# wujian16/Cornell-MOE

Measured on AMD Instinct MI355X. Metric: q-KG gradient evals/s (n=1000,d=8,q=4,10k MC), higher is better.
Workload: dtype f64

## Files before the change

cornell_moe_amd/_lib.py:

```python
import ctypes as C
import os

_HERE = os.path.dirname(os.path.abspath(__file__))
LIB_PATH = os.environ.get("MOE_LIB_PATH") or os.path.join(_HERE, "lib", "libmoe_hip.so")

dp = C.POINTER(C.c_double)
ip = C.POINTER(C.c_int)

MOE_OK, MOE_ERR_RUNTIME, MOE_ERR_BOUNDS, MOE_ERR_INVALID_VALUE, MOE_ERR_SINGULAR = 0, 1, 2, 3, 4
COV_SQUARE_EXPONENTIAL, COV_MATERN_NU_2P5 = 0, 1


class MoeError(C.Structure):
    _fields_ = [("code", C.c_int), ("message", C.c_char * 480), ("payload", C.c_double * 3)]


class GdParams(C.Structure):
    _fields_ = [("num_multistarts", C.c_int), ("max_num_steps", C.c_int), ("max_num_restarts", C.c_int),
                ("num_steps_averaged", C.c_int), ("gamma", C.c_double), ("pre_mult", C.c_double),
                ("max_relative_change", C.c_double), ("tolerance", C.c_double), ("domain_type", C.c_int)]


class Prior(C.Structure):
    _fields_ = [("kind", C.c_int), ("a", C.c_double), ("b", C.c_double)]
# ... 134 lines not shown
    "moe_ll_destroy": (C.c_int, [C.c_void_p]),
    "moe_ll_evaluate": (C.c_int, [C.c_void_p, dp, C.c_int, dp, _EP]),
    "moe_ll_grad": (C.c_int, [C.c_void_p, dp, dp, _EP]),
    "moe_ll_set_objective": (C.c_int, [C.c_void_p, C.c_int, _EP]),
    "moe_ll_get_objective": (C.c_int, [C.c_void_p]),
    "moe_ll_loo_predict": (C.c_int, [C.c_void_p, dp, dp, dp, _EP]),
    "moe_ll_ascend": (C.c_int, [C.c_void_p, C.POINTER(GdParams), dp, dp, dp, _EP]),
    "moe_ll_multistart": (C.c_int, [C.c_void_p, C.POINTER(GdParams), dp, dp, C.c_int, dp, dp, ip, _EP]),
    "moe_ll_mcmc": (C.c_int, [C.c_void_p, C.POINTER(Prior), C.c_int, C.c_int, C.c_double, dp, dp, ip, dp, dp, dp, dp, dp, ip, _EP]),
    "moe_posterior_mean_optimize": (C.c_int, [_GP, C.c_int, C.POINTER(GdParams), dp, dp, dp, dp, _EP]),
    "moe_latin_hypercube": (C.c_int, [C.c_uint, dp, C.c_int, C.c_int, dp]),
    "moe_gp_mix_covariance": (C.c_int, [_GP, dp, C.c_int, ip, C.c_int, dp, _EP]),
    "moe_cov_build_probe": (C.c_int, [_GP, dp, C.c_int, C.c_int, dp, dp, _EP]),
    "moe_debug_cholesky": (C.c_int, [C.c_int, dp, C.c_int, dp, dp, ip, _EP]),
    "moe_debug_math": (C.c_int, [C.c_int, dp, C.c_int, dp, dp, _EP]),
    "moe_kxx_build_probe": (C.c_int, [_GP, C.c_int, dp, dp, _EP]),
    "moe_debug_fp64_rate": (C.c_int, [C.c_int, dp, _EP]),
    "moe_set_reference_quirks": (C.c_int, [C.c_int]),
    "moe_get_reference_quirks": (C.c_int, []),
    "moe_set_ensemble_launches": (C.c_int, [C.c_int]),
    "moe_ensemble_launch_stats": (C.c_int, [C.POINTER(C.c_longlong)]),
    "moe_last_kernel_ms": (C.c_int, [_GP, dp]),
    "moe_last_kernel_info": (C.c_int, [_GP, C.POINTER(C.c_int)]),
}

_lib = None


def load():
    global _lib
    if _lib is None:
        if not os.path.exists(LIB_PATH):
            raise ImportError("%s is missing: run `python -m cornell_moe_amd.build` (needs hipcc); there is no CPU fallback"
                              % LIB_PATH)
        lib = C.CDLL(LIB_PATH)
        for name, (res, args) in SIGNATURES.items():
            fn = getattr(lib, name)
            fn.restype = res
            fn.argtypes = args
        _lib = lib
    return _lib


def device_count():
    n = C.c_int(0)
    load().moe_device_count(C.byref(n))
# ... 7 lines not shown
```

cornell_moe_amd/api.py:

```python
import ctypes as C

import numpy as np

from . import _lib
from ._lib import dp, ip


class OptimalLearningException(Exception):
    pass


class BoundsException(OptimalLearningException):
    def __init__(self, message, value=0.0, min=0.0, max=0.0):
        super(BoundsException, self).__init__(message)
        self.value, self.min, self.max = value, min, max


class InvalidValueException(OptimalLearningException):
    def __init__(self, message, value=0.0, truth=0.0, tolerance=0.0):
        super(InvalidValueException, self).__init__(message)
        self.value, self.truth, self.tolerance = value, truth, tolerance


class SingularMatrixException(OptimalLearningException):
# ... 526 lines not shown
        x0, xp = _d(initial_guess)
        out = np.zeros(self.d - num_fidelity)
        val = C.c_double(0.0)
        err = _lib.MoeError()
        _check(_lib.load().moe_posterior_mean_optimize(self._h, int(num_fidelity), C.byref(g), bp, xp, out.ctypes.data_as(dp),
                                                       C.byref(val), C.byref(err)), err)
        return out, val.value

    def last_kernel_ms(self):
        out = np.zeros(5)
        _lib.load().moe_last_kernel_ms(self._h, out.ctypes.data_as(dp))
        return dict(mc=out[0], cov_build=out[1], tail=out[2], state=out[3], total=out[4])


    def last_kernel_info(self):
        out = (C.c_int * 8)()
        _lib.load().moe_last_kernel_info(self._h, out)
        keys = ("variant", "xlds", "waves", "tr", "weight_table", "fused_tail", "blocks", "prep")
        info = dict(zip(keys, [int(v) for v in out]))
        info["far_frame"], info["wide_frame"], info["lane"] = (info["xlds"] >> 1) & 1, (info["xlds"] >> 2) & 1, (info["xlds"] >> 3) & 1
        info["start_table"] = (info["xlds"] >> 4) & 1
        info["xlds"] &= 1
        return info


def kg_batch_multi(gps, shard, inner_params, bounds, discrete, Xq_all, Xp, num_mc, best_so_far, normals, want_grad=True,
                   num_fidelity=0):
    L = _lib.load()
    g0 = gps[0]
    gd = DeviceGP._gd(inner_params)
    bounds, bp = _d(bounds)
    discrete, dpp = _d(discrete)
    P = discrete.reshape(-1, g0.d - num_fidelity).shape[0]
    Xq_all = np.ascontiguousarray(Xq_all, dtype=np.float64)
    R, q, _ = Xq_all.shape
    if Xp is None or np.size(Xp) == 0:
        p, ppp = 0, None
    else:
        Xp, ppp = _d(Xp)
        p = Xp.reshape(-1, g0.d).shape[0]
    normals, npn = _d(normals)
    arr = (C.c_void_p * len(gps))(*[g._h.value for g in gps])
    kg = np.zeros(R)
    grad = np.zeros(R * q * g0.d)
    stats = _lib.KgStats()
    err = _lib.MoeError()
# ... 759 lines not shown
```

cornell_moe_amd/csrc/api.hip:

```cpp
#include <memory>
#include <algorithm>
#include <cmath>
#include <cstring>
#include <functional>
#include <mutex>
#include <random>
#include <string>
#include <condition_variable>
#include <thread>

#include "gp.hpp"
#include "kg.hpp"
#include "kg1_ascent.hpp"

struct moe_gp {
  moe::GpDev dev;
  std::mutex mu;
  moe_gp(const double* hyper, int cov_type, const double* X, const double* y, const double* noise, const int* derivs, int g,
         int d, int n, int device)
      : dev(hyper, cov_type, X, y, noise, derivs, g, d, n, device) {}
};

namespace {

// ... 497 lines not shown
    moe::DevBuf<double> dx, de, dr;
    dx.upload(x, n, nullptr);
    de.reserve(n);
    dr.reserve(n);
    moe::launch_debug_math(dx.p, n, de.p, dr.p, nullptr);
    de.download(exp_neg, n, nullptr);
    dr.download(sqrt_out, n, nullptr);
    MOE_HIP_CHECK(hipStreamSynchronize(nullptr));
  });
}

int moe_last_kernel_ms(const moe_gp_t* gp, double* out5) {
  if (gp == nullptr || out5 == nullptr) return MOE_ERR_RUNTIME;
  std::lock_guard<std::mutex> lk(const_cast<moe_gp_t*>(gp)->mu);
  for (int i = 0; i < 5; ++i) out5[i] = gp->dev.last_ms[i];
  return MOE_OK;
}

int moe_last_kernel_info(const moe_gp_t* gp, int* out8) {
  if (gp == nullptr || out8 == nullptr) return MOE_ERR_RUNTIME;
  std::lock_guard<std::mutex> lk(const_cast<moe_gp_t*>(gp)->mu);
  for (int i = 0; i < 8; ++i) out8[i] = gp->dev.last_info[i];
  return MOE_OK;
}

int moe_ei(const moe_gp_t* gp_c, const double* points_to_sample, const double* points_being_sampled, int num_to_sample,
           int num_being_sampled, int num_mc, double best_so_far, const double* normals, double* ei, double* grad_ei,
           moe_error_t* err) {
  return guarded(err, [&] {
    std::unique_lock<std::mutex> lk;
    moe::GpDev& gp = lock_gp(gp_c, lk);
    moe::ei_evaluate(gp, points_to_sample, points_being_sampled, num_to_sample, num_being_sampled, num_mc, best_so_far,
                     normals, ei, grad_ei);
  });
}

int moe_ei_batch(const moe_gp_t* gp_c, const double* points_to_sample_all, int num_evals, const double* points_being_sampled,
                 int num_to_sample, int num_being_sampled, int num_mc, double best_so_far, const double* normals,
                 double* ei, double* grad_ei, moe_error_t* err) {
  return guarded(err, [&] {
    std::unique_lock<std::mutex> lk;
    moe::GpDev& gp = lock_gp(gp_c, lk);
    moe::ei_evaluate_batch(gp, points_to_sample_all, num_evals, points_being_sampled, num_to_sample, num_being_sampled, num_mc,
                           best_so_far, normals, ei, grad_ei);
  });
}
// ... 1351 lines not shown
```

cornell_moe_amd/csrc/gp.hpp:

```cpp
#pragma once
#include <cstdlib>
#include <functional>
#include <memory>
#include <vector>

#include "common.hpp"
#include "host_math.hpp"
#include "kernels.hpp"

namespace moe {

void fill_cov_params(CovParams& cp, int cov_type, int d, const double* hyper);

struct GpDev {
  int device = 0;
  hipStream_t stream = nullptr;
  hipStream_t side_stream = nullptr;
  void release_side_streams();
  int d = 0, dp = 0, n = 0, g = 0, N = 0;
  long ldL = 0;
  const double* zeroed_L = nullptr;
  long zeroed_ld = 0;
  CovParams cp;
  DerivList derivs;
// ... 18 lines not shown
  DevBuf<double> kStateD;
  DevBuf<double> sMat, sOut;
  DevBuf<int> sInfo;
  DevBuf<double> lcbD;
  DevBuf<int> lcbI;
  DevBuf<double> looD;
  DevBuf<double> kg1D;
  DevBuf<int> kg1I;
  int kg1LastC = 0;
  DevBuf<double> kg1oD;
  DevBuf<int> kg1oI;
  DevBuf<double> ehviD;
  DevBuf<double> recD;
  DevBuf<int> recI;
  DevBuf<double> pmmD;
  DevBuf<int> pmmI;
  DevBuf<double> pathD;
  DevBuf<int> pathI;
  int num_cu = 256;
  double x_mean[kMaxDimPadded] = {0}, x_ext[kMaxDimPadded] = {0};
  void refresh_extent();
  double last_ms[5] = {0, 0, 0, 0, 0};
  int last_info[8] = {0, 0, 0, 0, 0, 0, 0, 0};

  GpDev(const double* hyper, int cov_type, const double* X_in, const double* y_in, const double* noise_in,
        const int* derivs_in, int g_in, int d_in, int n_in, int device_in);
  ~GpDev();
  GpDev(const GpDev&) = delete;
  GpDev& operator=(const GpDev&) = delete;

  void use_device() const;
  void set_covariance(const double* hyper);
  void rebuild();
  void add_points(const double* pts, const double* vals, int k);
  void add_points_unchecked(const double* pts, const double* vals, int k);
  void finish_factorisation();
  void set_hyperparameters(const double* hyper, const double* noise_in);
  double log_marginal_likelihood();
  void grad_log_marginal_likelihood(double* grad);
  std::vector<double> padded(const double* pts, int k) const;
  void mean_of_points(const double* pts, int k, double* mu, double* grad);
};

struct StateDev {
  StateLayout lay;
  bool have_W = false;
// ... 142 lines not shown
```

cornell_moe_amd/csrc/kg.hip:

```cpp
#include "kg.hpp"

#include <algorithm>
#include <array>
#include <memory>
#include <optional>
#include <chrono>
#include <cmath>
#include <cstdlib>

#include "kg_mc.hpp"
#include "kg_prep.hpp"
#include "kg_state.hpp"
#include "kg_tail.hpp"

namespace moe {

static thread_local int t_ens_members_hint = 1;
int ensemble_members_hint() { return t_ens_members_hint; }
void set_ensemble_members_hint(int members) { t_ens_members_hint = members > 1 ? members : 1; }


namespace {

struct EventTimer {
  hipEvent_t a = nullptr, b = nullptr;
  bool on = false;
  EventTimer() = default;
  EventTimer(const EventTimer&) = delete;
  EventTimer& operator=(const EventTimer&) = delete;
  ~EventTimer() {
    if (a != nullptr) (void)hipEventDestroy(a);
    if (b != nullptr) (void)hipEventDestroy(b);
  }
  void start(hipStream_t s) {
    on = Recorder::current() == nullptr;
    if (!on) return;
    if (a == nullptr) {
      MOE_HIP_CHECK(hipEventCreate(&a));
      MOE_HIP_CHECK(hipEventCreate(&b));
    }
    MOE_HIP_CHECK(hipEventRecord(a, s));
  }
  void stop(hipStream_t s) {
    if (on) MOE_HIP_CHECK(hipEventRecord(b, s));
  }
// ... 68 lines not shown
}

struct McPlan {
  int G = 0;
  int ntiles = 0;
  int variant = 0;
  bool xlds = true;
  bool far_frame = false;
  bool wide_frame = false;
  bool small_lane = false;
  bool lane_kernel = false;
  int waves = 0, blocks = 0;
  size_t shm = 0;
  int tr = -1, num_lds_tiles = 0;
  int wide_lds_tiles = 0;
  int pair_rows = 0;
  int rec_head = 0;
  int multi_trial = 0;
  bool prep = false;
  bool start_table = false;
  bool weight_table = false;
  long v_stride = 0;
  int v_slots1 = 0;
  bool fused_tail = false;
  int chunk_len = 0;
};

McPlan plan_mc(const GpDev& gp, const KgDims& k, const double* bounds, const double* Xq_all, const double* Xp, double weight_table_gb) {
  const double max_radius2 = (double)env_int("MOE_KG_DOT_MAX_RADIUS2", 10000);
  const bool lane_on = env_int("MOE_KG_LANE", 1) != 0;
  const long small_lane_max_samples = env_int("MOE_KG_SMALL_LANE_MAX_SAMPLES", 1024);
  const bool small_multi = env_int("MOE_KG_SMALL_MULTI", 1) != 0;
  const std::optional<int> forced_tr = env_opt("MOE_KG_TR");
  const std::optional<int> forced_variant = env_opt("MOE_KG_VARIANT");
  const int prep_mode = env_int("MOE_KG_PREP", -1);
  const bool stream_weights = env_int("MOE_KG_STREAM_WEIGHTS", 1) != 0;
  const double v_cap = std::getenv("MOE_KG_V_MAX_GB") ? (double)env_int("MOE_KG_V_MAX_GB", 4)
                                                      : (weight_table_gb >= 0.0 ? weight_table_gb : 4.0);
  McPlan pl;
  pl.fused_tail = fused_tail_taken(k.want_grad, k.g, k.m);

  const int d = k.d, dp = k.dp, n = k.n, g = k.g, m = k.m, u = k.u, A = k.A, E = k.E, num_local = k.num_local;
  const bool wide_dp = dp > 16;
  const int G = wide_dp ? (g == 0 ? 0 : (g <= 4 ? 4 : (g <= 8 ? 8 : 12))) : (g <= 4 ? g : (g <= 8 ? 8 : 12));
  const int ntiles = (n + u + 63) / 64;

  const size_t tab_bytes = sizeof(double) * (size_t)ntiles * (dp + 1) * 64;
  const size_t slab_bytes = sizeof(double) * ((size_t)ntiles * (1 + G) * 64 + 2 * kMaxM);
  const size_t slab_stream_bytes = slab_bytes + (mc::wide_eval(dp, false) ? sizeof(double) * mc::kWideScratch : 0);
  const size_t pad_bytes = sizeof(double) * (size_t)(1 + G) * 64;
  const size_t fixed_bytes = sizeof(double) * (kExpTabLen + (size_t)mc::kCstRows * dp);
  const size_t lds_max = 160 * 1024 - fixed_bytes - pad_bytes;
  bool xlds = true;
  bool wide_frame = false, far_frame = false;
  {
    double rad2 = 0.0;
    for (int kk = 0; kk < d; ++kk) {
      const double c = gp.x_mean[kk];
      double ext = gp.x_ext[kk];
// ... 92 lines not shown
  }
  if (ensemble_members_hint() > 1 && variant != 1 && blocks >= E && waves > 0) {
    const long tickets = 4;
    const long kb = std::max<long>(1, (num_local + tickets * waves - 1) / (tickets * waves));
    blocks = (int)std::min<long>(blocks, kb * E);
  }

  pl.G = G;
  pl.ntiles = ntiles;
  pl.variant = variant;
  pl.xlds = xlds;
  pl.far_frame = far_frame;
  pl.wide_frame = wide_frame;
  pl.small_lane = small_lane;
  pl.lane_kernel = lane_kernel;
  pl.waves = waves;
  pl.blocks = blocks;
  pl.shm = shm;
  pl.tr = tr;
  pl.num_lds_tiles = num_lds_tiles;
  pl.wide_lds_tiles = wide_lds_tiles;
  pl.pair_rows = (wide_dp || variant == 2 || (variant == 0 && mc::wide_eval(dp, xlds))) ? 1 : 0;
  pl.rec_head = rec_head;
  pl.multi_trial = (far_frame || small_lane) ? 0 : 1;
  if (small_lane && !far_frame && variant == 0 && lane_kernel && dp == 4 && small_multi) pl.multi_trial = 2;
  pl.prep = m > kMaxM || (prep_mode != 0 && (variant >= 1 || prep_mode == 1));
  pl.v_stride = (variant == 2) ? v_stride_tiles : k.N;
  pl.v_slots1 = (variant == 2) ? 1 + G : k.g1;
  pl.weight_table = variant >= 1 && pl.prep && 8.0 * (double)pl.v_stride * (double)num_local / 1e9 <= v_cap;
  if (variant == 2 && !(pl.weight_table && pl.prep))
    throw Error(MOE_ERR_RUNTIME, "streamed-weights MC kernel selected without its weight table");
  pl.chunk_len = tail_chunk_len(pl.fused_tail, m);
  pl.start_table = variant == 0 && xlds && g == 0 && G == 0;
  return pl;
}

TabParams table_rows(const GpDev& gp, const KgDims& k, int G, const double* Xq_all, const double* Xp, const double* disc_head) {
  const int d = k.d;
  TabParams tp;
  std::vector<int> order;
  std::vector<bool> used(kMaxDimPadded, false);
  for (int a = 0; a < k.g; ++a) {
    if (used[gp.derivs.idx[a]]) throw Error(MOE_ERR_INVALID_VALUE, "duplicate derivative index", gp.derivs.idx[a], 0, 0);
    order.push_back(gp.derivs.idx[a]);
    used[gp.derivs.idx[a]] = true;
  }
// ... 172 lines not shown
  mp.max_num_restarts = gd.max_num_restarts;
  mp.gamma = gd.gamma;
  mp.pre_mult = gd.pre_mult;
  mp.max_relative_change = gd.max_relative_change;
  if (k.simplex && mp.max_relative_change == 1.0) mp.max_relative_change -= 4.0 * 2.220446049250313e-16;
  mp.simplex = k.simplex ? 1 : 0;
  mp.inv_sqrt_size = 1.0 / std::sqrt((double)k.size);
  for (int r = 0; r < kMaxDimPadded; ++r) mp.inv_perm[r] = 0;
  for (int r = 0; r < kMaxDimPadded; ++r)
    if (tp.perm[r] >= 0 && tp.perm[r] < kMaxDimPadded) mp.inv_perm[tp.perm[r]] = r;
  mp.tolerance = gd.tolerance;
  mp.best_point = gp.kBestPoint.p;
  mp.best_value = gp.kBestValue.p;
  mp.beta = gp.kBeta.p;
  mp.counters = gp.kCounters.p;
  mp.next_sample = reinterpret_cast<unsigned int*>(gp.kCounters.p + (((size_t)2 * E + 15) / 16) * 16);
  mp.prof = gp.kCounters.p + n_ctr - 16;
  mp.best_j = nullptr;
  mp.V = nullptr;
  mp.v_stride = pl.v_stride;
  mp.v_slots1 = pl.v_slots1;
  mp.start_tab = nullptr;
  mp.start_stride = 0;
  if (pl.start_table) {
    mp.start_stride = (long)k.A * (1 + m) * (dp + 1);
    gp.kStartTab.reserve((size_t)mp.start_stride * E);
    double* start_tab_p = gp.kStartTab.p;
    launch_start_table(mp, dp, start_tab_p, s);
    mp.start_tab = start_tab_p;
  }
  t_state.stop(s);
  t_mc.start(s);
  const long total = (long)E * num_local;
  if (pl.prep) {
    gp.kBestJ.reserve((size_t)total);
    mp.best_j = gp.kBestJ.p;
    launch_sample_prep(mp, gp.kBestJ.p, gp.num_cu, s);
  }
  if (pl.weight_table) {
    gp.kV.reserve((size_t)mp.v_stride * (size_t)total + (size_t)64 * mp.v_slots1);
    memset_async(gp.kBeta.p + (size_t)total * m, 0, sizeof(double) * 64, s);
    mp.V = gp.kV.p;
    launch_sample_weights(mp, gp.kV.p, s, pl.variant == 2);
  }
  if (pl.variant == 0 && pl.lane_kernel)
    launch_mc_lane(mp, dp, pl.G, pl.rec_head, pl.blocks, pl.waves, pl.shm, s);
// ... 275 lines not shown
  gp.kBeta.reserve((size_t)E * num_local * m + 64);
  const size_t n_ctr = (size_t)2 * E + (size_t)E * (kTicketStride / 2) + 32;
  gp.kCounters.reserve(n_ctr);
  const int out_stride = 1 + m * m + 2 * k.ngrad;
  gp.kOut.reserve((size_t)out_stride * E);
  const bool sw_free = pl.fused_tail && fused_tail_sw_free();
  if (want_grad) {
    const int chunks = (num_local + pl.chunk_len - 1) / pl.chunk_len;
    if (!pl.fused_tail) gp.kT.reserve((size_t)N * E * num_local);
    if (!sw_free) gp.kC.reserve((size_t)E * num_local * m);
    gp.kTB.reserve((size_t)E * (chunks + 1) * m * N + (size_t)E * k.ngrad * kDirSlices + (sw_free ? (size_t)E * chunks * m * m : 0));
  }

  launch_xs_tab(gp.dX.p, k.n, gp.dUnion, u, dp, pl.ntiles, tp, gp.kTab.p, tab_stride, pl.pair_rows, gp.kCounters.p, (long)n_ctr, E, s);

  const KgMcParams mp = launch_mc_step(gp, k, pl, gd, tp, R, dBlobP, dNormalsP, se.bl, tab_stride, n_ctr, t_state, t_mc, s);
  {
    const int info[8] = {pl.variant,
                         ((pl.variant == 0 && pl.xlds) ? 1 : 0) | (pl.far_frame ? 2 : 0) | (pl.wide_frame ? 4 : 0) | (pl.lane_kernel ? 8 : 0) |
                             (pl.start_table ? 16 : 0),
                         pl.waves, pl.variant == 1 ? pl.tr : pl.wide_lds_tiles, pl.weight_table ? 1 : 0, pl.fused_tail ? 1 : 0, pl.blocks,
                         pl.prep ? 1 : 0};
    std::copy(info, info + 8, gp.last_info);
  }

  const KgTailParams tl = launch_tail_step(gp, k, pl, mp, R, dBlobP, dNormalsP, se.bl, dFin, out_stride, t_cov, t_tail, s);
  if (want_grad) {
    launch_grad_finish(gp, k, sp, tl, R, dBlobP, dFin, out_stride, sw_free, s);
    t_tail.stop(s);
  }
  return enqueue_results(gp, k, dFin, n_ctr, want_best_points, timers, wall0, s);
}

int kg_max_batch(const GpDev& gp, int P, int q, int p, int num_local, bool want_grad, double budget_gb) {
  const double N = gp.N, g1 = 1 + gp.g, u = q + p, m = u * g1, A = u + P;
  const double ngrad = want_grad ? q * g1 * gp.d : 0.0;
  const bool fused = fused_tail_taken(want_grad, gp.g, (int)m);
  const double chunks = std::ceil((double)num_local / tail_chunk_len(fused, (int)m));
  double doubles = N * (m + ngrad + A) + 3.0 * N * m + (double)num_local * (gp.dp + 1 + 2 * m) +
                   (want_grad ? (double)q * gp.d * m * (m + 1) / 2 : 0.0);
  if (want_grad) doubles += (fused ? 0.0 : N * (double)num_local) + (chunks + 1.0) * m * N;
  if (want_grad && !fused) doubles += 9.0 * m * (double)num_local;
  const double slots1 = gp.g <= 4 ? g1 : (gp.g <= 8 ? 9.0 : 13.0);
  doubles += (gp.n + u + 64.0) * slots1 * (double)num_local;
  doubles += 8.0 * N * m + (m * m + A * (1.0 + m + gp.d) + u * gp.dp + 8.0);
  const double per_eval_gb = 8.0 * doubles / 1e9;
// ... 33 lines not shown
```

cornell_moe_amd/csrc/kg_mc.hpp:

```cpp
#pragma once
#include <hip/hip_runtime.h>

#include "fastmath.hpp"
#include "kernels.hpp"

namespace moe {

#ifndef MOE_BLOCK_PROF
#define MOE_BLOCK_PROF 0
#endif
#if MOE_BLOCK_PROF
#define MOE_PROF_T(var) const unsigned long long var = __builtin_amdgcn_s_memtime()
#define MOE_PROF_ADD(dst, a, b) dst += (b) - (a)
#else
#define MOE_PROF_T(var)
#define MOE_PROF_ADD(dst, a, b)
#endif
constexpr int kTicketStride = 32;
constexpr int kMaxM = 64;
constexpr int kMaxMB = 128;
constexpr int kExpTabLen = 64;

struct KgRec {
  int L;
// ... 23 lines not shown
  const double* KinvY;
  const double* W;
  long w_stride;
  const double* blob;
  KgRec rec;
  const double* bounds;
  unsigned int free_mask;
  const double* normals;
  int first_sample, num_local;
  int max_num_steps, max_num_restarts;
  double gamma, pre_mult, max_relative_change, tolerance;
  double* best_point;
  double* best_value;
  double* beta;
  unsigned long long* counters;
  unsigned int* next_sample;
  unsigned long long* prof;
  const double* V;
  long v_stride;
  int v_slots1;
  const int* best_j;
  const double* start_tab;
  long start_stride;
};

#if defined(__HIPCC__)
namespace mc {

template <int DP> void launch_dp(const KgMcParams& P, int G, bool xlds, int blocks, int waves, size_t shm, hipStream_t s);
template <int DP> void launch_lane_dp(const KgMcParams& P, int G, int rec_head, int blocks, int waves, size_t shm, hipStream_t s);
template <int DP> void launch_stream_dp(const KgMcParams& P, int G, int blocks, int waves, size_t shm, hipStream_t s);
template <int DP> void launch_block_dp(const KgMcParams& P, int G, int tr, int num_lds_tiles, int blocks, int waves, hipStream_t s);

template <int CTRL, int ROW_MASK, bool FULL>
__device__ __forceinline__ double dpp_move(double v) {
  const int slo = __double2loint(v), shi = __double2hiint(v);
  int lo, hi;
  if (FULL) {
    lo = __builtin_amdgcn_mov_dpp(slo, CTRL, ROW_MASK, 0xf, false);
    hi = __builtin_amdgcn_mov_dpp(shi, CTRL, ROW_MASK, 0xf, false);
  } else {
    lo = __builtin_amdgcn_update_dpp(0, slo, CTRL, ROW_MASK, 0xf, false);
    hi = __builtin_amdgcn_update_dpp(0, shi, CTRL, ROW_MASK, 0xf, false);
  }
  return __hiloint2double(hi, lo);
}

// ... 729 lines not shown
      const double* Cj = C_disc + (long)j * m;
      for (int c0 = 0; c0 < m; c0 += 8) {
        double cv[8];
#pragma unroll
        for (int i = 0; i < 8; ++i) cv[i] = Cj[min(c0 + i, m - 1)];
#pragma unroll
        for (int i = 0; i < 8; ++i) v = fma(cv[i], (c0 + i < m) ? zb[min(c0 + i, kMaxM - 1)] : 0.0, v);
      }
      fj = -v;
    }
    double wmax = fj;
#pragma unroll
    for (int off = 32; off > 0; off >>= 1) wmax = fmax(wmax, __shfl_xor(wmax, off, 64));
    const unsigned long long ballot = __ballot(fj == wmax);
    const int first_lane = __ffsll((long long)ballot) - 1;
    if (wmax > best_f) {
      best_f = wmax;
      best_j = j0 + first_lane;
    }
  }
  return __builtin_amdgcn_readfirstlane(best_j);
}

}

inline size_t kg_mc_block_lds_bytes(int dp, int G, int num_lds_tiles) {
  return sizeof(double) * (mc::kBlockFixed + (size_t)num_lds_tiles * (dp + 1 + G) * 64);
}
inline size_t kg_mc_lane_fixed_bytes(int dp, int rec_head) {
  return sizeof(double) * ((size_t)kExpTabLen + (size_t)mc::kLaneCstRows * dp + (size_t)((rec_head + 1) & ~1));
}

#endif

}
```

cornell_moe_amd/csrc/kg_mc_block.hpp:

```cpp
#pragma once
#include "kg_mc.hpp"
#include "kg_mc_lds.hpp"

namespace moe {
namespace mc {


template <int DP, int G, bool WG, int COV>
__device__ __forceinline__ void point_terms(const double (&cx)[DP], const double (&cw)[1 + G], const double (&xq)[DP],
                                            const double* __restrict__ etab, double& accf, double (&accg)[DP],
                                            double (&accd)[G > 0 ? G : 1]) {
  double diff[DP];
  double r2 = 1.0e-300;
#pragma unroll
  for (int k = 0; k < DP; ++k) {
    diff[k] = cx[k] - xq[k];
    r2 = fma(diff[k], diff[k], r2);
  }
  double base, first, second;
  radial3<COV, (WG || G > 0), (WG && G > 0)>(r2, etab, base, first, second);
  double sd = 0.0;
  if (G > 0) {
#pragma unroll
    for (int a = 0; a < G; ++a) sd = fma(cw[1 + a], diff[a], sd);
// ... 489 lines not shown
    double* ldsw = ldsx + (long)num_lds_tiles * DP * 64;
    const int lane = threadIdx.x & 63;
    const int wave = threadIdx.x >> 6;
    const int nw = blockDim.x >> 6;
    const int m = P.m;
    const int size = P.dim - P.f;
    const int TL = num_lds_tiles;
    const int per = (TL + nw - 1) / nw;
    const int tl0 = min(wave * per, TL), tl1 = min(tl0 + per, TL);
    if (threadIdx.x < kExpTabLen) etab[threadIdx.x] = kExp2Tab64[threadIdx.x];
    BlockEval<DP, G, TR> ev;
    ev.xl = ldsx + (long)tl0 * DP * 64 + lane;
    ev.wl = ldsw + (long)tl0 * (1 + G) * 64 + lane;
    ev.ntl = tl1 - tl0;
    ev.etab = etab;
    ev.part = part;
    ev.inv_lp = P.inv_lp;
    ev.mean = P.mean;
    ev.nw = nw;
    ev.wave = wave;
    ev.lane = lane;
    ev.cov_type = P.cov_type;
    ev.par = 0;
    for (int e = blockIdx.x % P.E; e < P.E; e += (gridDim.x < (unsigned)P.E ? gridDim.x : P.E)) {
      const double* tab = P.XsTab + (long)e * P.tab_stride;
      const double* rec = P.blob + (long)e * P.rec.stride;
      const double* Lsm = rec + P.rec.L;
      const double* We = P.W + (long)e * P.w_stride;
      __syncthreads();
      if constexpr (DP > 16) {
        for (int t = threadIdx.x; t < TL * DP * 64; t += blockDim.x) {
          const int l = t & 63, r = (t >> 6) % DP, tile = (t >> 6) / DP;
          ldsx[t] = tab[(((long)tile * (DP / 2) + (r >> 1)) * 64 + l) * 2 + (r & 1)];
        }
      } else {
        for (int t = threadIdx.x; t < TL * DP * 64; t += blockDim.x) ldsx[t] = tab[t];
      }
  #pragma unroll
      for (int t = 0; t < TR; ++t) {
        const int tile = TL + wave * TR + t;
  #pragma unroll
        for (int k = 0; k < DP; ++k) ev.cx[t][k] = (tile < P.ntiles) ? tab[((long)tile * DP + k) * 64 + lane] : 0.0;
      }
  #if MOE_BLOCK_PROF
      unsigned long long p_tick = 0, p_setup = 0, p_w = 0, p_ls = 0, p_zb = 0, p_scan = 0;
  #endif
      while (true) {
// ... 83 lines not shown
          if (P.best_j == nullptr && lane < m) P.beta[so * m + lane] = bc;
        }
      }
  #if MOE_BLOCK_PROF
      if (threadIdx.x == 0) {
        atomicAdd(&P.prof[0], p_tick);
        atomicAdd(&P.prof[1], p_setup);
        atomicAdd(&P.prof[2], p_w);
        atomicAdd(&P.prof[3], p_ls);
        atomicAdd(&P.prof[4], ev.c_acc);
        atomicAdd(&P.prof[5], ev.c_red);
        atomicAdd(&P.prof[6], ev.c_bar);
        atomicAdd(&P.prof[7], ev.c_post);
        atomicAdd(&P.prof[8], ev.c_n);
        atomicAdd(&P.prof[9], ev.c_gtot);
        atomicAdd(&P.prof[10], ev.c_gn);
        atomicAdd(&P.prof[11], p_zb);
        atomicAdd(&P.prof[12], p_scan);
        atomicAdd(&P.prof[13], ev.seg[0]);
        atomicAdd(&P.prof[14], ev.seg[1]);
        atomicAdd(&P.prof[15], ev.seg[2] + ev.seg[3]);
      }
  #endif
      if (gridDim.x >= (unsigned)P.E) break;
    }
  }
};
template <int DP, int G, int TR>
__global__ __launch_bounds__(512) void kg_mc_block_kernel(KgMcParams P, int num_lds_tiles) {
  kg_mc_block_kernel_body<DP, G, TR>::run(MOE_VBLOCK, MOE_VGRID, nullptr, P, num_lds_tiles);
}

template <int DP, int G, int TR>
inline void launch_block_inst(const KgMcParams& P, int num_lds_tiles, int blocks, int waves, hipStream_t s) {
  const size_t shm = sizeof(double) * (kBlockFixed + (size_t)num_lds_tiles * (DP + 1 + G) * 64);
  auto kern = kg_mc_block_kernel<DP, G, TR>;
  launch_kernel_ens<kg_mc_block_kernel_body<DP, G, TR>, 512>(kern, dim3(blocks), dim3(waves * 64), shm, s, P, num_lds_tiles);
  MOE_HIP_CHECK(hipGetLastError());
}

template <int DP, int G>
inline void launch_block_g(const KgMcParams& P, int tr, int num_lds_tiles, int blocks, int waves, hipStream_t s) {
  switch (tr) {
    case 0: return launch_block_inst<DP, G, 0>(P, num_lds_tiles, blocks, waves, s);
    case 2: if constexpr (DP <= 16) return launch_block_inst<DP, G, 2>(P, num_lds_tiles, blocks, waves, s); break;
    case 4: if constexpr (DP <= 16) return launch_block_inst<DP, G, 4>(P, num_lds_tiles, blocks, waves, s); break;
  }
// ... 23 lines not shown
```

cornell_moe_amd/csrc/kg_mc_lane.hpp:

```cpp
#pragma once
#include "kg_mc.hpp"

namespace moe {
namespace mc {

constexpr int kLaneMaxThreads = 512;
constexpr int kLaneGradUnroll = 4;

template <int DP, int G, bool EXACT>
constexpr bool kLaneLookupFirst = DP <= 8 && G <= 1 && !EXACT;

constexpr int kMaxLaneDP = 16;

template <int DP>
__device__ __forceinline__ void fill_lane_constants(const KgMcParams& P, double* __restrict__ cst) {
  const int r = threadIdx.x;
  if (r < DP) {
    const double sc = P.inv_lp[r];
    cst[r] = sc;
    cst[DP + r] = (sc != 0.0) ? 1.0 / sc : 0.0;
    cst[2 * DP + r] = P.center[r];
    cst[3 * DP + r] = (P.perm[r] < P.dim) ? 1.0 : 0.0;
    cst[4 * DP + r] = P.bounds[2 * r];
    cst[5 * DP + r] = P.bounds[2 * r + 1];
// ... 443 lines not shown
  tot_val += n_val;
  tot_grad += n_grad;
  if (in_l) P.best_point[so * DP + perm_l] = xo_l;
  if (lane < m) P.beta[so * m + lane] = bc;
}

template <int DP, int G, bool EXACT = false, bool LF = false>
struct kg_mc_lane_kernel_body {
static __device__ __forceinline__ void run(const VIdx blockIdx, const VIdx gridDim, const void* argbase, const KgMcParams& P, int rec_head) {
  extern __shared__ __attribute__((aligned(16))) double smem[];
  const int lane = threadIdx.x & 63;
  const int wave = threadIdx.x >> 6;
  const int ntiles = P.ntiles;
  const int tab = ntiles * (DP + 1) * 64;
  const int wslab = ntiles * (1 + G) * 64 + 2 * kMaxM;
  double* cst = smem + kExpTabLen;
  double* rc = cst + kLaneCstRows * DP;
  double* coords = rc + rec_head;
  double* wshared = coords + tab;
  double* aw = wshared + wave * wslab;
  double* zb = aw + ntiles * (1 + G) * 64;
  if (threadIdx.x < kExpTabLen) smem[threadIdx.x] = kExp2Tab64[threadIdx.x];
  fill_lane_constants<DP>(P, cst);
  for (int e = blockIdx.x % P.E; e < P.E; e += (gridDim.x < (unsigned)P.E ? gridDim.x : P.E)) {
    const double* xg = P.XsTab + (long)e * P.tab_stride;
    __syncthreads();
    for (int pt = threadIdx.x; pt < ntiles * 64; pt += blockDim.x) {
      const int tl = pt >> 6, l = pt & 63;
      const double* src = xg + (long)tl * DP * 64 + l;
      double* dst = coords + tl * (DP + 1) * 64 + l;
      double xx = 0.0;
#pragma unroll
      for (int k = 0; k < DP; ++k) {
        const double v = src[k * 64];
        dst[k * 64] = v;
        xx = fma(v, v, xx);
      }
      dst[DP * 64] = xx;
    }
    {
      const double* rec = P.blob + (long)e * P.rec.stride;
      for (int i = threadIdx.x; i < rec_head; i += blockDim.x) rc[i] = rec[i];
    }
    __syncthreads();
    unsigned int ticket = 0;
    unsigned int* next = P.next_sample + (long)e * kTicketStride;
    if (lane == 0) ticket = atomicAdd(next, 1u);
    unsigned int tot_val = 0, tot_grad = 0;
    while (true) {
      const unsigned int sl = (unsigned int)__builtin_amdgcn_readfirstlane((int)ticket);
      if (sl >= (unsigned int)P.num_local) break;
      if (lane == 0) ticket = atomicAdd(next, 1u);
      const __attribute__((address_space(4))) KgMcParams* Pk = (const __attribute__((address_space(4))) KgMcParams*)argbase;
      asm volatile("" : "+s"(Pk));
      kg_sample_lane<DP, G, EXACT, LF>(*(const KgMcParams*)Pk, e, (int)sl, coords, aw, zb, smem, cst, rc, lane, tot_val, tot_grad);
    }
    if (lane == 0 && (tot_val | tot_grad) != 0) {
      atomicAdd(&P.counters[2 * e], (unsigned long long)tot_val);
      atomicAdd(&P.counters[2 * e + 1], (unsigned long long)tot_grad);
    }
    if (gridDim.x >= (unsigned)P.E) break;
  }
}
};
template <int DP, int G, bool EXACT = false>
__global__ __launch_bounds__(kLaneMaxThreads) void kg_mc_lane_kernel(KgMcParams P, int rec_head) {
  kg_mc_lane_kernel_body<DP, G, EXACT, kLaneLookupFirst<DP, G, EXACT>>::run(MOE_VBLOCK, MOE_VGRID, (const void*)__builtin_amdgcn_kernarg_segment_ptr(), P, rec_head);
}

template <int DP, int G, bool EXACT = false>
inline void launch_lane_inst(const KgMcParams& P, int rec_head, int blocks, int waves, size_t shm, hipStream_t s) {
  auto kern = kg_mc_lane_kernel<DP, G, EXACT>;
  launch_kernel_ens<kg_mc_lane_kernel_body<DP, G, EXACT>, kLaneMaxThreads>(kern, dim3(blocks), dim3(waves * 64), shm, s, P, rec_head);
  MOE_HIP_CHECK(hipGetLastError());
}

template <int DP, int G>
inline void launch_lane_g(const KgMcParams& P, int rec_head, int blocks, int waves, size_t shm, hipStream_t s) {
  if constexpr (DP == 4) {
    if (P.multi_trial == 2) return launch_lane_inst<DP, G, true>(P, rec_head, blocks, waves, shm, s);
  }
  launch_lane_inst<DP, G>(P, rec_head, blocks, waves, shm, s);
}

// ... 17 lines not shown
```

cornell_moe_amd/csrc/kg_mc_stream.hpp:

```cpp
#pragma once
#include "kg_mc.hpp"
#include "kg_mc_lds.hpp"

namespace moe {
namespace mc {

template <int DP, int G>
struct kg_mc_stream_kernel_body {
  static __device__ __forceinline__ void run(const VIdx blockIdx, const VIdx gridDim, const void*, const KgMcParams& P) {
    extern __shared__ __attribute__((aligned(16))) double smem[];
    const int lane = threadIdx.x & 63;
    const int wave = threadIdx.x >> 6;
    const int wtab = P.wide_lds_tiles * DP * 64;
    double* coords = smem + kExpTabLen;
    double* st = coords + wtab + wave * kWideScratch;
    if (threadIdx.x < kExpTabLen) smem[threadIdx.x] = kExp2Tab64[threadIdx.x];
    const int size = P.dim - P.f;
    for (int e = blockIdx.x % P.E; e < P.E; e += (gridDim.x < (unsigned)P.E ? gridDim.x : P.E)) {
      const double* xs = P.XsTab + (long)e * P.tab_stride;
      const double* rec = P.blob + (long)e * P.rec.stride;
      __syncthreads();
      {
        const d2t* src = reinterpret_cast<const d2t*>(xs);
        d2t* dst = reinterpret_cast<d2t*>(coords);
        for (int i = threadIdx.x; i < wtab / 2; i += blockDim.x) dst[i] = src[i];
      }
      __syncthreads();
      unsigned int ticket = 0;
      unsigned int* next = P.next_sample + (long)e * kTicketStride;
      if (lane == 0) ticket = atomicAdd(next, 1u);
      unsigned long long tot_val = 0, tot_grad = 0;
      while (true) {
        const unsigned int sl = (unsigned int)__builtin_amdgcn_readfirstlane((int)ticket);
        if (sl >= (unsigned int)P.num_local) break;
        if (lane == 0) ticket = atomicAdd(next, 1u);
        const long so = (long)e * P.num_local + sl;
        const int best_j = P.best_j[so];
        const double* disc = rec + P.rec.disc;
        double x[DP];
  #pragma unroll
        for (int k = 0; k < DP; ++k) x[k] = (k < size) ? disc[(long)best_j * size + k] : ((k < P.dim) ? 1.0 : 0.0);
        const d2t* xg = reinterpret_cast<const d2t*>(xs) + lane;
        lds_pair_ptr xl = (lds_pair_ptr)coords + lane;
        WideEval<DP, G, true> ev{xg, xl, {P.V + so * P.v_stride + (long)lane * (1 + G)}, smem, st + kLsRows * kMaxDimPadded,
                                 P.ntiles, P.wide_lds_tiles, P.cov_type, lane, P.mean};
        unsigned long long n_val = 0, n_grad = 0;
        const double fcur = line_search_lds<DP, G>(P, ev, st, x, n_val, n_grad);
        if (lane == 0) P.best_value[so] = fcur;
        tot_val += n_val;
        tot_grad += n_grad;
        if (lane < DP) {
          double v = 0.0;
  #pragma unroll
          for (int k = 0; k < DP; ++k)
            if (lane == k) v = x[k];
          P.best_point[so * DP + lane] = v;
        }
      }
      if (lane == 0 && (tot_val | tot_grad) != 0) {
        atomicAdd(&P.counters[2 * e], tot_val);
        atomicAdd(&P.counters[2 * e + 1], tot_grad);
      }
      if (gridDim.x >= (unsigned)P.E) break;
    }
  }
};
template <int DP, int G>
__global__ __launch_bounds__(512) void kg_mc_stream_kernel(KgMcParams P) {
  kg_mc_stream_kernel_body<DP, G>::run(MOE_VBLOCK, MOE_VGRID, nullptr, P);
}

template <int DP, int G>
inline void launch_stream_inst(const KgMcParams& P, int blocks, int waves, size_t shm, hipStream_t s) {
  auto kern = kg_mc_stream_kernel<DP, G>;
  launch_kernel_ens<kg_mc_stream_kernel_body<DP, G>, 512>(kern, dim3(blocks), dim3(waves * 64), shm, s, P);
  MOE_HIP_CHECK(hipGetLastError());
}

template <int DP>
void launch_stream_dp(const KgMcParams& P, int G, int blocks, int waves, size_t shm, hipStream_t s) {
  switch (G) {
    case 0: return launch_stream_inst<DP, 0>(P, blocks, waves, shm, s);
    case 1: if constexpr (DP <= 16) return launch_stream_inst<DP, 1>(P, blocks, waves, shm, s); break;
    case 2: if constexpr (DP <= 16) return launch_stream_inst<DP, 2>(P, blocks, waves, shm, s); break;
    case 3: if constexpr (DP <= 16) return launch_stream_inst<DP, 3>(P, blocks, waves, shm, s); break;
    case 4: return launch_stream_inst<DP, 4>(P, blocks, waves, shm, s);
// ... 9 lines not shown
```

cornell_moe_amd/csrc/kg_mc_wave.hpp:

```cpp
#pragma once
#include "kg_mc.hpp"
#include "kg_mc_lds.hpp"

namespace moe {
namespace mc {

template <int DP, int G, bool SMALL, bool XL>
struct WaveEval {
  const double* __restrict__ xs;
  const double* __restrict__ aw;
  const double* __restrict__ etab;
  int ntiles, cov_type;
  double mean;
  int lane;
  double* __restrict__ scr;
#if MOE_BLOCK_PROF
  unsigned long long c_v = 0, c_g = 0, n_v = 0, n_g = 0;
#endif
  __device__ __forceinline__ double eval_grad_frame(const double (&xf)[DP], double (&gradf)[DP]) {
#if MOE_BLOCK_PROF
    const unsigned long long t0 = __builtin_amdgcn_s_memtime();
#endif
    const double f = eval_pass<DP, G, true, SMALL, XL>(xs, aw, etab, ntiles, cov_type, mean, xf, gradf, lane, scr);
#if MOE_BLOCK_PROF
// ... 388 lines not shown
      if (lane == k) v = x[k];
    P.best_point[so * DP + lane] = v;
  }
  if (!prepped && lane < m) P.beta[so * m + lane] = bc;
}

template <int DP, int G, bool XLDS, bool SMALL>
struct kg_mc_kernel_body {
  static __device__ __forceinline__ void run(const VIdx blockIdx, const VIdx gridDim, const void*, const KgMcParams& P) {
    extern __shared__ __attribute__((aligned(16))) double smem[];
    const int lane = threadIdx.x & 63;
    const int wave = threadIdx.x >> 6;
    const int ntiles = P.ntiles;
    const int tab = ntiles * (DP + 1) * 64;
    const int wslab = ntiles * (1 + G) * 64 + 2 * kMaxM + (wide_eval(DP, XLDS) ? kWideScratch : 0);
    double* cst = smem + kExpTabLen;
    double* coords = cst + kCstRows * DP;
    const int wtab = wide_eval(DP, XLDS) ? P.wide_lds_tiles * DP * 64 : 0;
    double* aw = coords + (XLDS ? tab : wtab) + wave * wslab;
    double* zb = aw + ntiles * (1 + G) * 64;
    if (threadIdx.x < kExpTabLen) smem[threadIdx.x] = kExp2Tab64[threadIdx.x];
    fill_frame_constants<DP>(P, cst);
    if (!XLDS) __syncthreads();
    for (int e = blockIdx.x % P.E; e < P.E; e += (gridDim.x < (unsigned)P.E ? gridDim.x : P.E)) {
      const double* xs = P.XsTab + (long)e * P.tab_stride;
      if (XLDS) {
        __syncthreads();
        for (int pt = threadIdx.x; pt < ntiles * 64; pt += blockDim.x) {
          const int tl = pt >> 6, l = pt & 63;
          const double* src = xs + (long)tl * DP * 64 + l;
          double* dst = coords + tl * (DP + 1) * 64 + l;
          double xx = 0.0;
  #pragma unroll
          for (int k = 0; k < DP; ++k) {
            const double v = src[k * 64];
            dst[k * 64] = v;
            xx = fma(v, v, xx);
          }
          dst[DP * 64] = xx;
        }
        xs = coords;
        __syncthreads();
      }
      if constexpr (wide_eval(DP, XLDS)) {
        __syncthreads();
        const d2t* src = reinterpret_cast<const d2t*>(xs);
        d2t* dst = reinterpret_cast<d2t*>(coords);
        for (int i = threadIdx.x; i < wtab / 2; i += blockDim.x) dst[i] = src[i];
        __syncthreads();
      }
      unsigned int ticket = 0;
      unsigned int* next = P.next_sample + (long)e * kTicketStride;
      if (lane == 0) ticket = atomicAdd(next, 1u);
      unsigned long long tot_val = 0, tot_grad = 0;
      while (true) {
        const unsigned int sl = (unsigned int)__builtin_amdgcn_readfirstlane((int)ticket);
        if (sl >= (unsigned int)P.num_local) break;
        if (lane == 0) ticket = atomicAdd(next, 1u);
        kg_sample<DP, G, SMALL, XLDS>(P, e, (int)sl, xs, aw, zb, smem, cst, lane, tot_val, tot_grad);
      }
      if (lane == 0 && (tot_val | tot_grad) != 0) {
        atomicAdd(&P.counters[2 * e], tot_val);
        atomicAdd(&P.counters[2 * e + 1], tot_grad);
      }
      if (gridDim.x >= (unsigned)P.E) break;
    }
  }
};
template <int DP, int G, bool XLDS, bool SMALL>
__global__ __launch_bounds__(SMALL ? 1024 : 512) void kg_mc_kernel(KgMcParams P) {
  kg_mc_kernel_body<DP, G, XLDS, SMALL>::run(MOE_VBLOCK, MOE_VGRID, nullptr, P);
}

template <int DP, int G, bool XLDS, bool SMALL>
inline void launch_inst2(const KgMcParams& P, int blocks, int waves, size_t shm, hipStream_t s) {
  auto kern = kg_mc_kernel<DP, G, XLDS, SMALL>;
  launch_kernel_ens<kg_mc_kernel_body<DP, G, XLDS, SMALL>, (SMALL ? 1024 : 512)>(kern, dim3(blocks), dim3(waves * 64), shm, s, P);
  MOE_HIP_CHECK(hipGetLastError());
}

template <int DP, int G>
inline void launch_g(const KgMcParams& P, bool xlds, int blocks, int waves, size_t shm, hipStream_t s) {
  if constexpr (DP <= 16) {
    if (xlds && waves > 8) return launch_inst2<DP, G, true, true>(P, blocks, waves, shm, s);
    if (xlds) return launch_inst2<DP, G, true, false>(P, blocks, waves, shm, s);
  }
  launch_inst2<DP, G, false, false>(P, blocks, waves, shm, s);
}
// ... 19 lines not shown
```

include/moe_hip.h:

```cpp
#ifndef MOE_HIP_H_
#define MOE_HIP_H_

#ifdef __cplusplus
extern "C" {
#endif

#define MOE_OK 0
#define MOE_ERR_RUNTIME 1
#define MOE_ERR_BOUNDS 2
#define MOE_ERR_INVALID_VALUE 3
#define MOE_ERR_SINGULAR 4

#define MOE_COV_SQUARE_EXPONENTIAL 0
#define MOE_COV_MATERN_NU_2P5 1

typedef struct moe_error {
  int code;
  char message[480];
  double payload[3];
} moe_error_t;

typedef struct moe_gd_params {
  int num_multistarts;
  int max_num_steps;
// ... 310 lines not shown
#define MOE_PRIOR_FIXED 5
typedef struct moe_prior {
  int kind;
  double a, b;
} moe_prior_t;
int moe_ll_mcmc(moe_ll_t* ll, const moe_prior_t* priors, int num_walkers, int num_steps, double stretch_a, const double* p0,
                const double* u_stretch, const int* partner, const double* u_accept, double* chain, double* lnprob, double* lnprob0,
                double* proposal_lnprob, int* accepted, moe_error_t* err);

int moe_gp_mix_covariance(const moe_gp_t* gp, const double* pts, int num_pts, const int* derivs2, int g2, double* out,
                          moe_error_t* err);
int moe_cov_build_probe(const moe_gp_t* gp, const double* pts, int num_pts, int repeat, double* avg_ms,
                        double* bytes_per_launch, moe_error_t* err);

int moe_kxx_build_probe(const moe_gp_t* gp, int repeat, double* avg_ms, double* bytes_per_launch, moe_error_t* err);
int moe_debug_fp64_rate(int device, double* tflops, moe_error_t* err);

int moe_debug_cholesky(int n, const double* a, int device, double* chol, double* chol_inv, int* info, moe_error_t* err);

int moe_debug_math(int n, const double* x, int device, double* exp_neg, double* sqrt_out, moe_error_t* err);

int moe_last_kernel_ms(const moe_gp_t* gp, double* out5);
int moe_last_kernel_info(const moe_gp_t* gp, int* out8);

#ifdef __cplusplus
}
#endif
#endif
```

Measured before the change: 2026.

## Let KG Monte Carlo blocks steal samples from the evaluation with most remaining work

After finishing its assigned evaluation (or its strided sequence of them), a block scans the per-evaluation ticket counters, picks the evaluation with the most undrawn samples, and joins it through the existing atomic ticket loop. The goal is to reduce tail imbalance where some evaluations finish early and leave compute units idle while others still have many samples. It adds a global scan with atomics and extra block syncs per move, plus a moves counter and debug accessors for moves and best points. It is on by default via MOE_KG_STEAL.

```diff
diff --git a/cornell_moe_amd/_lib.py b/cornell_moe_amd/_lib.py
--- a/cornell_moe_amd/_lib.py
+++ b/cornell_moe_amd/_lib.py
@@ -180,6 +180,8 @@
     "moe_ensemble_launch_stats": (C.c_int, [C.POINTER(C.c_longlong)]),
     "moe_last_kernel_ms": (C.c_int, [_GP, dp]),
     "moe_last_kernel_info": (C.c_int, [_GP, C.POINTER(C.c_int)]),
+    "moe_last_kg_moves": (C.c_int, [_GP, C.POINTER(C.c_longlong)]),
+    "moe_last_kg_best_points": (C.c_int, [_GP, C.POINTER(C.c_int), C.POINTER(C.c_int), dp, C.c_longlong]),
 }
 
 _lib = None
diff --git a/cornell_moe_amd/api.py b/cornell_moe_amd/api.py
--- a/cornell_moe_amd/api.py
+++ b/cornell_moe_amd/api.py
@@ -572,6 +572,22 @@
         info["start_table"] = (info["xlds"] >> 4) & 1
         info["xlds"] &= 1
         return info
+
+    def last_kg_moves(self):
+        out = C.c_longlong(0)
+        if _lib.load().moe_last_kg_moves(self._h, C.byref(out)):
+            raise RuntimeError("moe_last_kg_moves failed")
+        return int(out.value)
+
+    def last_kg_best_points(self):
+        L = _lib.load()
+        E, M = C.c_int(0), C.c_int(0)
+        if L.moe_last_kg_best_points(self._h, C.byref(E), C.byref(M), None, 0):
+            raise RuntimeError("moe_last_kg_best_points failed")
+        out = np.zeros((E.value, M.value, self.d))
+        if out.size and L.moe_last_kg_best_points(self._h, C.byref(E), C.byref(M), out.ctypes.data_as(dp), out.size):
+            raise RuntimeError("moe_last_kg_best_points failed")
+        return out
 
 
 def kg_batch_multi(gps, shard, inner_params, bounds, discrete, Xq_all, Xp, num_mc, best_so_far, normals, want_grad=True,
diff --git a/cornell_moe_amd/csrc/api.hip b/cornell_moe_amd/csrc/api.hip
--- a/cornell_moe_amd/csrc/api.hip
+++ b/cornell_moe_amd/csrc/api.hip
@@ -543,6 +543,41 @@
   std::lock_guard<std::mutex> lk(const_cast<moe_gp_t*>(gp)->mu);
   for (int i = 0; i < 8; ++i) out8[i] = gp->dev.last_info[i];
   return MOE_OK;
+}
+
+int moe_last_kg_moves(const moe_gp_t* gp_c, long long* moves) {
+  if (gp_c == nullptr || moves == nullptr) return MOE_ERR_RUNTIME;
+  return guarded(nullptr, [&] {
+    std::unique_lock<std::mutex> lk;
+    moe::GpDev& gp = lock_gp(gp_c, lk);
+    unsigned long long w = 0;
+    if (gp.last_moves != nullptr) {
+      gp.use_device();
+      MOE_HIP_CHECK(hipStreamSynchronize(gp.stream));
+      MOE_HIP_CHECK(hipMemcpy(&w, gp.last_moves, sizeof(w), hipMemcpyDeviceToHost));
+    }
+    *moves = (long long)w;
+  });
+}
+
+int moe_last_kg_best_points(const moe_gp_t* gp_c, int* num_evals, int* num_local, double* out, long long capacity) {
+  if (gp_c == nullptr || num_evals == nullptr || num_local == nullptr) return MOE_ERR_RUNTIME;
+  return guarded(nullptr, [&] {
+    std::unique_lock<std::mutex> lk;
+    moe::GpDev& gp = lock_gp(gp_c, lk);
+    const int E = gp.last_best_shape[0], M = gp.last_best_shape[1], d = gp.d, dp = gp.dp;
+    *num_evals = E;
+    *num_local = M;
+    const size_t rows = (size_t)E * M;
+    if (out == nullptr || rows == 0) return;
+    require(capacity >= (long long)(rows * d), "moe_last_kg_best_points: output too small");
+    gp.use_device();
+    MOE_HIP_CHECK(hipStreamSynchronize(gp.stream));
+    std::vector<double> padded(rows * dp);
+    MOE_HIP_CHECK(hipMemcpy(padded.data(), gp.kBestPoint.p, sizeof(double) * padded.size(), hipMemcpyDeviceToHost));
+    for (size_t i = 0; i < rows; ++i)
+      for (int k = 0; k < d; ++k) out[i * d + k] = padded[i * dp + k];
+  });
 }
 
 int moe_ei(const moe_gp_t* gp_c, const double* points_to_sample, const double* points_being_sampled, int num_to_sample,
diff --git a/cornell_moe_amd/csrc/gp.hpp b/cornell_moe_amd/csrc/gp.hpp
--- a/cornell_moe_amd/csrc/gp.hpp
+++ b/cornell_moe_amd/csrc/gp.hpp
@@ -64,6 +64,8 @@
   void refresh_extent();
   double last_ms[5] = {0, 0, 0, 0, 0};
   int last_info[8] = {0, 0, 0, 0, 0, 0, 0, 0};
+  const unsigned long long* last_moves = nullptr;
+  int last_best_shape[2] = {0, 0};
 
   GpDev(const double* hyper, int cov_type, const double* X_in, const double* y_in, const double* noise_in,
         const int* derivs_in, int g_in, int d_in, int n_in, int device_in);
diff --git a/cornell_moe_amd/csrc/kg.hip b/cornell_moe_amd/csrc/kg.hip
--- a/cornell_moe_amd/csrc/kg.hip
+++ b/cornell_moe_amd/csrc/kg.hip
@@ -21,6 +21,8 @@
 
 
 namespace {
+
+constexpr int kStealWaves = 2;
 
 struct EventTimer {
   hipEvent_t a = nullptr, b = nullptr;
@@ -135,6 +137,8 @@
   bool weight_table = false;
   long v_stride = 0;
   int v_slots1 = 0;
+  int steal_min = 0;
+  int steal_skew = 0;
   bool fused_tail = false;
   int chunk_len = 0;
 };
@@ -148,6 +152,8 @@
   const std::optional<int> forced_variant = env_opt("MOE_KG_VARIANT");
   const int prep_mode = env_int("MOE_KG_PREP", -1);
   const bool stream_weights = env_int("MOE_KG_STREAM_WEIGHTS", 1) != 0;
+  const bool steal = env_int("MOE_KG_STEAL", 1) != 0;
+  const bool steal_skew = env_int("MOE_KG_STEAL_SKEW", 0) != 0;
   const double v_cap = std::getenv("MOE_KG_V_MAX_GB") ? (double)env_int("MOE_KG_V_MAX_GB", 4)
                                                       : (weight_table_gb >= 0.0 ? weight_table_gb : 4.0);
   McPlan pl;
@@ -286,6 +292,9 @@
   pl.wide_lds_tiles = wide_lds_tiles;
   pl.pair_rows = (wide_dp || variant == 2 || (variant == 0 && mc::wide_eval(dp, xlds))) ? 1 : 0;
   pl.rec_head = rec_head;
+  if (steal_skew && !steal) throw Error(MOE_ERR_INVALID_VALUE, "MOE_KG_STEAL_SKEW=1 needs MOE_KG_STEAL=1", 0, 0, 0);
+  pl.steal_min = !steal ? 0 : (steal_skew ? 1 : std::max(1, env_int("MOE_KG_STEAL_MIN_PER_WAVE", kStealWaves) * (variant == 1 ? 1 : waves)));
+  pl.steal_skew = steal_skew ? 1 : 0;
   pl.multi_trial = (far_frame || small_lane) ? 0 : 1;
   if (small_lane && !far_frame && variant == 0 && lane_kernel && dp == 4 && small_multi) pl.multi_trial = 2;
   pl.prep = m > kMaxM || (prep_mode != 0 && (variant >= 1 || prep_mode == 1));
@@ -504,6 +513,8 @@
   mp.v_slots1 = pl.v_slots1;
   mp.start_tab = nullptr;
   mp.start_stride = 0;
+  mp.steal_min = pl.steal_min;
+  mp.steal_skew = pl.steal_skew;
   if (pl.start_table) {
     mp.start_stride = (long)k.A * (1 + m) * (dp + 1);
     gp.kStartTab.reserve((size_t)mp.start_stride * E);
@@ -825,6 +836,9 @@
                          pl.waves, pl.variant == 1 ? pl.tr : pl.wide_lds_tiles, pl.weight_table ? 1 : 0, pl.fused_tail ? 1 : 0, pl.blocks,
                          pl.prep ? 1 : 0};
     std::copy(info, info + 8, gp.last_info);
+    gp.last_moves = mp.prof + kMovesWord;
+    gp.last_best_shape[0] = E;
+    gp.last_best_shape[1] = k.num_local;
   }
 
   const KgTailParams tl = launch_tail_step(gp, k, pl, mp, R, dBlobP, dNormalsP, se.bl, dFin, out_stride, t_cov, t_tail, s);
diff --git a/cornell_moe_amd/csrc/kg_mc.hpp b/cornell_moe_amd/csrc/kg_mc.hpp
--- a/cornell_moe_amd/csrc/kg_mc.hpp
+++ b/cornell_moe_amd/csrc/kg_mc.hpp
@@ -69,7 +69,10 @@
   const int* best_j;
   const double* start_tab;
   long start_stride;
+  int steal_min;
+  int steal_skew;
 };
+constexpr int kMovesWord = 15;
 
 #if defined(__HIPCC__)
 namespace mc {
@@ -845,6 +848,51 @@
   return __builtin_amdgcn_readfirstlane(best_j);
 }
 
+__device__ __forceinline__ int first_evaluation(const KgMcParams& P, const VIdx& blockIdx) {
+  return P.steal_skew != 0 ? 0 : (int)(blockIdx.x % (unsigned)P.E);
+}
+__device__ __forceinline__ int move_to_fullest(const unsigned int* next_sample, unsigned long long* moves, int E, int num_local,
+                                            int steal_min, int e, int* slot) {
+  __syncthreads();
+  if (threadIdx.x < 64) {
+    const int lane = threadIdx.x;
+    unsigned long long key = 0;
+    for (int c = lane; c < E; c += 64) {
+      const unsigned int drawn = __hip_atomic_load(next_sample + (long)c * kTicketStride, __ATOMIC_RELAXED, __HIP_MEMORY_SCOPE_AGENT);
+      const unsigned int nl = (unsigned int)num_local;
+      const unsigned int remaining = nl - min(drawn, nl);
+      int dist = c - e - 1;
+      if (dist < 0) dist += E;
+      const unsigned long long k2 = ((unsigned long long)remaining << 32) | (0xffffffffu - (unsigned int)dist);
+      key = k2 > key ? k2 : key;
+    }
+#pragma unroll
+    for (int off = 32; off > 0; off >>= 1) {
+      const unsigned long long o = __shfl_xor(key, off, 64);
+      key = o > key ? o : key;
+    }
+    if (lane == 0) {
+      const unsigned int remaining = (unsigned int)(key >> 32);
+      const int dist = (int)(0xffffffffu - (unsigned int)key);
+      const int to = (remaining >= (unsigned int)steal_min) ? (e + 1 + dist) % E : -1;
+      *(volatile int*)slot = to;
+#if !MOE_BLOCK_PROF
+      if (to >= 0) atomicAdd(moves, 1ull);
+#endif
+    }
+  }
+  __syncthreads();
+  const int to = __builtin_amdgcn_readfirstlane(*(volatile int*)slot);
+  __syncthreads();
+  return to;
+}
+__device__ __forceinline__ int next_evaluation(const KgMcParams& P, const VIdx& gridDim, int e, bool& moved, int* slot) {
+  if (!moved && P.steal_skew == 0 && gridDim.x < (unsigned)P.E && e + (int)gridDim.x < P.E) return e + (int)gridDim.x;
+  if (P.steal_min <= 0 || P.E == 1) return -1;
+  moved = true;
+  return move_to_fullest(P.next_sample, P.prof + kMovesWord, P.E, P.num_local, P.steal_min, e, slot);
+}
+
 }
 
 inline size_t kg_mc_block_lds_bytes(int dp, int G, int num_lds_tiles) {
diff --git a/cornell_moe_amd/csrc/kg_mc_block.hpp b/cornell_moe_amd/csrc/kg_mc_block.hpp
--- a/cornell_moe_amd/csrc/kg_mc_block.hpp
+++ b/cornell_moe_amd/csrc/kg_mc_block.hpp
@@ -535,7 +535,8 @@
     ev.lane = lane;
     ev.cov_type = P.cov_type;
     ev.par = 0;
-    for (int e = blockIdx.x % P.E; e < P.E; e += (gridDim.x < (unsigned)P.E ? gridDim.x : P.E)) {
+    bool moved = false;
+    for (int e = first_evaluation(P, blockIdx); e >= 0; e = next_evaluation(P, gridDim, e, moved, ctl)) {
       const double* tab = P.XsTab + (long)e * P.tab_stride;
       const double* rec = P.blob + (long)e * P.rec.stride;
       const double* Lsm = rec + P.rec.L;
@@ -665,7 +666,6 @@
         atomicAdd(&P.prof[15], ev.seg[2] + ev.seg[3]);
       }
   #endif
-      if (gridDim.x >= (unsigned)P.E) break;
     }
   }
 };
diff --git a/cornell_moe_amd/csrc/kg_mc_lane.hpp b/cornell_moe_amd/csrc/kg_mc_lane.hpp
--- a/cornell_moe_amd/csrc/kg_mc_lane.hpp
+++ b/cornell_moe_amd/csrc/kg_mc_lane.hpp
@@ -489,7 +489,9 @@
   double* zb = aw + ntiles * (1 + G) * 64;
   if (threadIdx.x < kExpTabLen) smem[threadIdx.x] = kExp2Tab64[threadIdx.x];
   fill_lane_constants<DP>(P, cst);
-  for (int e = blockIdx.x % P.E; e < P.E; e += (gridDim.x < (unsigned)P.E ? gridDim.x : P.E)) {
+  bool moved = false;
+  for (int e = first_evaluation(P, blockIdx); e >= 0;
+       e = next_evaluation(P, gridDim, e, moved, reinterpret_cast<int*>(wshared + ntiles * (1 + G) * 64))) {
     const double* xg = P.XsTab + (long)e * P.tab_stride;
     __syncthreads();
     for (int pt = threadIdx.x; pt < ntiles * 64; pt += blockDim.x) {
@@ -526,7 +528,6 @@
       atomicAdd(&P.counters[2 * e], (unsigned long long)tot_val);
       atomicAdd(&P.counters[2 * e + 1], (unsigned long long)tot_grad);
     }
-    if (gridDim.x >= (unsigned)P.E) break;
   }
 }
 };
diff --git a/cornell_moe_amd/csrc/kg_mc_stream.hpp b/cornell_moe_amd/csrc/kg_mc_stream.hpp
--- a/cornell_moe_amd/csrc/kg_mc_stream.hpp
+++ b/cornell_moe_amd/csrc/kg_mc_stream.hpp
@@ -16,7 +16,8 @@
     double* st = coords + wtab + wave * kWideScratch;
     if (threadIdx.x < kExpTabLen) smem[threadIdx.x] = kExp2Tab64[threadIdx.x];
     const int size = P.dim - P.f;
-    for (int e = blockIdx.x % P.E; e < P.E; e += (gridDim.x < (unsigned)P.E ? gridDim.x : P.E)) {
+    bool moved = false;
+    for (int e = first_evaluation(P, blockIdx); e >= 0; e = next_evaluation(P, gridDim, e, moved, reinterpret_cast<int*>(coords + wtab))) {
       const double* xs = P.XsTab + (long)e * P.tab_stride;
       const double* rec = P.blob + (long)e * P.rec.stride;
       __syncthreads();
@@ -61,7 +62,6 @@
         atomicAdd(&P.counters[2 * e], tot_val);
         atomicAdd(&P.counters[2 * e + 1], tot_grad);
       }
-      if (gridDim.x >= (unsigned)P.E) break;
     }
   }
 };
diff --git a/cornell_moe_amd/csrc/kg_mc_wave.hpp b/cornell_moe_amd/csrc/kg_mc_wave.hpp
--- a/cornell_moe_amd/csrc/kg_mc_wave.hpp
+++ b/cornell_moe_amd/csrc/kg_mc_wave.hpp
@@ -434,7 +434,9 @@
     if (threadIdx.x < kExpTabLen) smem[threadIdx.x] = kExp2Tab64[threadIdx.x];
     fill_frame_constants<DP>(P, cst);
     if (!XLDS) __syncthreads();
-    for (int e = blockIdx.x % P.E; e < P.E; e += (gridDim.x < (unsigned)P.E ? gridDim.x : P.E)) {
+    bool moved = false;
+    for (int e = first_evaluation(P, blockIdx); e >= 0;
+         e = next_evaluation(P, gridDim, e, moved, reinterpret_cast<int*>(coords + (XLDS ? tab : wtab) + ntiles * (1 + G) * 64))) {
       const double* xs = P.XsTab + (long)e * P.tab_stride;
       if (XLDS) {
         __syncthreads();
@@ -475,7 +477,6 @@
         atomicAdd(&P.counters[2 * e], tot_val);
         atomicAdd(&P.counters[2 * e + 1], tot_grad);
       }
-      if (gridDim.x >= (unsigned)P.E) break;
     }
   }
 };
diff --git a/include/moe_hip.h b/include/moe_hip.h
--- a/include/moe_hip.h
+++ b/include/moe_hip.h
@@ -356,6 +356,8 @@
 
 int moe_last_kernel_ms(const moe_gp_t* gp, double* out5);
 int moe_last_kernel_info(const moe_gp_t* gp, int* out8);
+int moe_last_kg_moves(const moe_gp_t* gp, long long* moves);
+int moe_last_kg_best_points(const moe_gp_t* gp, int* num_evals, int* num_local, double* out, long long capacity);
 
 #ifdef __cplusplus
 }
```

After: 2140, median of 6. 5.6% higher.
